# sile/libflate

Measured on AMD Instinct MI355X. Metric: gzip encode+decode throughput on 256 MiB synthetic text per GPU (uncompressed bytes through the round trip), higher is better.
Workload: dtype u8; 1 GPU; cfg2: gzip::Encoder (DefaultLz77Encoder, default options, mtime=0) + gzip::Decoder on TEXT(268435456 B) per GPU, write schedule S8K (8192-byte writes); bytes_per_gpu=268435456, schedule=S8K, compressed_bytes=129579521, parallelism=1 rank

## Files before the change

### libflate_amd/csrc/lfx_inflate_fast.hip

```cpp
#include <hip/hip_runtime.h>
#include <stdint.h>
#include <stdlib.h>

#include <type_traits>

#include "lfx_common.h"
#include "lfx_decode.h"

namespace lfx {

__constant__ uint16_t f_len_base[29] = {3,  4,  5,  6,  7,  8,  9,  10, 11,  13,  15,  17,  19,  23, 27,
                                        31, 35, 43, 51, 59, 67, 83, 99, 115, 131, 163, 195, 227, 258};
__constant__ uint8_t f_len_extra[29] = {0, 0, 0, 0, 0, 0, 0, 0, 1, 1, 1, 1, 2, 2, 2,
                                        2, 3, 3, 3, 3, 4, 4, 4, 4, 5, 5, 5, 5, 0};
__constant__ uint16_t f_dist_base[30] = {1,    2,    3,    4,    5,    7,    9,    13,    17,    25,
                                         33,   49,   65,   97,   129,  193,  257,  385,   513,   769,
                                         1025, 1537, 2049, 3073, 4097, 6145, 8193, 12289, 16385, 24577};
__constant__ uint8_t f_dist_extra[30] = {0, 0, 0, 0, 1, 1, 2, 2,  3,  3,  4,  4,  5,  5,  6,
                                         6, 7, 7, 8, 8, 9, 9, 10, 10, 11, 11, 12, 12, 13, 13};
__constant__ uint8_t f_clen_order[19] = {16, 17, 18, 0, 8, 7, 9, 6, 10, 5, 11, 4, 12, 3, 13, 2, 14, 1, 15};
constexpr uint32_t f_clen_order_c(uint32_t k) {
    constexpr uint8_t o[19] = {16, 17, 18, 0, 8, 7, 9, 6, 10, 5, 11, 4, 12, 3, 13, 2, 14, 1, 15};
    return o[k];
}
// ... 1057 lines not shown
                __syncthreads();
                uint32_t rounds = 0, no = 0, flag = 4;
                int32_t rr = INT32_MAX;
                uint64_t exitpos = ~0ull, decoded_from = ~0ull;
                for (;;) {
                    const uint64_t st = s_start[tid];
                    if (tid < nl && st != ~0ull) {
                        if (st != decoded_from) {
                            const int r = lane_count_reach(T, in, nb, st, tid + 1 == nl ? e : my_bound, no, rr, exitpos);
                            flag = r == 1 ? 1 : r == 2 ? 2 : 0;
                            decoded_from = st;
                        }
                    } else flag = 4;
                    s_flag[tid] = flag; s_exit[tid] = exitpos;
                    __syncthreads();
                    bool changed = false;
                    if (tid + 1 < nl && flag == 0 && s_start[tid + 1] != exitpos) { s_start[tid + 1] = exitpos; changed = true; }
                    rounds++;
                    const int any = __syncthreads_or(changed ? 1 : 0);
                    if (!any || rounds >= 64) break;
                }
                if (rounds >= 64) { fail = true; break; }
                if (tid < nl && s_flag[tid] != 0) atomicMin(&s_eob, tid);
                __syncthreads();
                uint32_t eobl = s_eob;
                if (eobl == 0xFFFFFFFFu) eobl = nl - 1;
                else if (s_flag[eobl] != 1) { fail = true; break; }
                else closed = true;
                const uint64_t myno = tid <= eobl ? no : 0;
                uint64_t y = myno;
                for (int o = 1; o < 64; o <<= 1) {
                    const uint64_t c = __shfl_up(y, o);
                    if ((int)lane >= o) y += c;
                }
                if (lane == 63) s_sum[wave] = y;
                __syncthreads();
                uint64_t py = 0, tot = 0;
                for (uint32_t w = 0; w < NT / 64; ++w) { const uint64_t s = s_sum[w]; py += w < wave ? s : 0; tot += s; }
                long long m = tid <= eobl && rr != INT32_MAX ? (long long)(produced + py + y - myno) + (long long)rr : INT64_MAX;
                for (int o = 32; o; o >>= 1) { const long long c = __shfl_xor(m, o); m = c < m ? c : m; }
                if (lane == 0) s_min[wave] = m;
                const uint64_t last_exit = s_exit[eobl];
                __syncthreads();
                for (uint32_t w = 0; w < NT / 64; ++w) { const long long c = s_min[w]; reach = c < reach ? c : reach; }
                produced += tot;
                if (closed) blk_end = last_exit;
                else if (last_exit <= w0 || last_exit >= end_bits) fail = true;
                else w0 = last_exit;
                __syncthreads();
            }
            if (fail) { produced = blk_out; break; }
        }
        if (blk_end <= cur || blk_end > end_bits) { produced = blk_out; break; }
        nblocks++;
        cur = blk_end;
        if (bfinal) { status = WALK_FINAL; break; }
        if (job.stop_bit && cur >= job.stop_bit) { status = WALK_STOP; break; }
        __syncthreads();
    }
    if (tid == 0) {
        WalkResult r;
        r.end_bit = cur; r.n_out = produced; r.stuck_bit = blk_bit; r.stuck_out = blk_out;
        r.reach = reach; r.status = status; r.nblocks = nblocks;
        results[blockIdx.x] = r;
    }
}

constexpr uint32_t MAX_UNITS = 8;

template <int NT = SCAN_THREADS>
__device__ __forceinline__ void blk_units_tail(const uint32_t tid, const BlkEmit &job, const BlkLanes *L, const int64_t reach,
                                               uint32_t cut_code, const uint64_t cut_pos, BlkUnits *U, const uint32_t unit_target,
                                               const uint32_t free_shift, const uint64_t t_begin, const uint64_t t_hdr) {
    const uint64_t t_dec = clock64();
    __shared__ int64_t s_wmin[NT / 64];
    const uint32_t lane = tid & 63, wave = tid >> 6;
    int64_t sfx = reach;
    for (int o = 1; o < 64; o <<= 1) {
        const int64_t y = __shfl_down(sfx, o);
        if (lane + o < 64 && y < sfx) sfx = y;
    }
    if (lane == 0) s_wmin[wave] = sfx;
    __syncthreads();
    int64_t later = __shfl_down(sfx, 1);
    if (lane == 63) later = INT64_MAX;
    for (uint32_t w = wave + 1; w < NT / 64; ++w) { const int64_t y = s_wmin[w]; if (y < later) later = y; }
    if (cut_code != 0xFFFFFFFFu && later < (int64_t)cut_pos) cut_code = 0xFFFFFFFFu;
    __shared__ uint32_t s_cut_code[NT];
    __shared__ uint64_t s_cut_pos[NT];
    s_cut_code[tid] = cut_code;
    s_cut_pos[tid] = cut_pos;
    __shared__ uint64_t s_legal[NT / 64];
    const uint64_t legal = __ballot(cut_code != 0xFFFFFFFFu);
    if (lane == 0) s_legal[wave] = legal;
    __syncthreads();
    const uint64_t t_cut = clock64();
    if (tid == 0) {
        uint32_t nu = 0, last = 0;
        uint32_t want_units = (job.n_codes + unit_target / 2) / unit_target;
        if (want_units < 1) want_units = 1;
        if (want_units > MAX_UNITS) want_units = MAX_UNITS;
        const uint32_t tol = job.n_codes / (2 * want_units);
        U->code0[0] = 0; U->out0[0] = 0;
        for (uint32_t b = 1; b < want_units; ++b) {
            const uint32_t ideal = (uint32_t)((uint64_t)job.n_codes * b / want_units);
            uint32_t l0 = (uint32_t)((uint64_t)job.nlanes * b / want_units);
            if (l0 >= NT) l0 = NT - 1;
            int up = -1, dn = -1;
            for (uint32_t w = l0 >> 6; w < NT / 64 && up < 0; ++w) {
                uint64_t m = s_legal[w];
                if (w == (l0 >> 6)) m &= ~0ull << (l0 & 63);
                if (m) up = (int)(w * 64 + (uint32_t)__builtin_ctzll(m));
            }
            for (int w = (int)(l0 >> 6); w >= 0 && dn < 0; --w) {
                uint64_t m = s_legal[w];
                if (w == (int)(l0 >> 6)) m &= (l0 & 63) ? ~0ull >> (64 - (l0 & 63)) : 0ull;
                if (m) dn = w * 64 + 63 - __builtin_clzll(m);
            }
            int pick = -1;
            uint32_t best = 0xFFFFFFFFu;
            if (up >= 0) { const uint32_t cc = s_cut_code[up]; const uint32_t d = cc > ideal ? cc - ideal : ideal - cc; if (d < best) { best = d; pick = up; } }
            if (dn >= 0) { const uint32_t cc = s_cut_code[dn]; const uint32_t d = cc > ideal ? cc - ideal : ideal - cc; if (d < best) { best = d; pick = dn; } }
            if (pick < 0 || best > tol) continue;
            const uint32_t cc = s_cut_code[pick];
            if (cc == 0 || cc <= last || cc >= job.n_codes) continue;
            nu++;
            U->code0[nu] = cc; U->out0[nu] = s_cut_pos[pick];
            last = cc;
        }
        nu++;
        U->code0[nu] = job.n_codes; U->out0[nu] = job.n_out;
        U->n = nu;
        uint32_t fn = 0;
        uint32_t fwant = (uint32_t)(job.n_out >> free_shift);
        fwant = fwant < 1 ? 1 : fwant > MAX_FREE_UNITS ? MAX_FREE_UNITS : fwant;
        U->fcode0[0] = 0; U->fout0[0] = 0;
        for (uint32_t b = 1; b < fwant; ++b) {
            const uint32_t l = (uint32_t)((uint64_t)job.nlanes * b / fwant);
            if (l == 0 || l >= job.nlanes) continue;
            const uint32_t cc = L->code_off[l];
            if (cc <= U->fcode0[fn] || cc >= job.n_codes) continue;
            fn++;
            U->fcode0[fn] = cc; U->fout0[fn] = L->out_off[l];
        }
        fn++;
        U->fcode0[fn] = job.n_codes; U->fout0[fn] = job.n_out;
        U->fn = fn;
        U->cyc[0] = (uint32_t)(t_hdr - t_begin); U->cyc[1] = (uint32_t)(t_dec - t_hdr);
        U->cyc[2] = (uint32_t)(t_cut - t_dec); U->cyc[3] = (uint32_t)(clock64() - t_cut);
    }
}

__device__ __forceinline__ void blk_flag_reach(uint32_t tid, int64_t reach, uint64_t hist, uint32_t *__restrict__ flags,
                                               uint32_t *__restrict__ job_flags) {
    __shared__ uint32_t s_fl;
    if (tid == 0) s_fl = 0;
    __syncthreads();
    if (reach < -(int64_t)hist) atomicOr(&s_fl, 1u);
    else if (reach < 0) atomicOr(&s_fl, 2u);
    __syncthreads();
    if (tid == 0 && s_fl) {
        const uint32_t f = s_fl;
        if ((f & 1u) && job_flags) job_flags[blockIdx.x] = 1u;
        if ((__atomic_load_n(&flags[0], __ATOMIC_RELAXED) & f) != f) atomicOr(&flags[0], f);
    }
}

template <bool RING, int NT = SCAN_THREADS>
__global__ __launch_bounds__(NT, RING ? 4 : 8) void blk_emit_kernel(const uint8_t *__restrict__ in, uint64_t nbytes,
                                                                const BlkEmit *__restrict__ jobs,
                                                                const BlkLanes *__restrict__ lanes,
                                                                uint32_t *__restrict__ codes,
                                                                uint32_t *__restrict__ flags,
                                                                BlkUnits *__restrict__ units, uint32_t unit_target, uint32_t free_shift,
                                                                uint32_t *__restrict__ job_flags,
                                                                const FastTabs *__restrict__ tabs) {
    __shared__ FastTabs T;
    __shared__ __attribute__((aligned(4))) uint8_t lens[640];
    __shared__ uint32_t hdr[8];
    __shared__ uint64_t hdr64[2];
    extern __shared__ uint32_t emit_stage[];
    __shared__ uint32_t s_ring[RING ? NT * RING_STRIDE : 1];
    const uint32_t tid = threadIdx.x;
    const BlkEmit job = jobs[blockIdx.x];
    BlkUnits *U = &units[blockIdx.x];
    if (job.placed) return;
    if (job.btype == 0) {
        if (tid == 0) {
            U->n = 1; U->code0[0] = 0; U->code0[1] = 0; U->out0[0] = 0; U->out0[1] = job.n_out;
            U->fn = 1; U->fcode0[0] = 0; U->fcode0[1] = 0; U->fout0[0] = 0; U->fout0[1] = job.n_out;
        }
        return;
    }
    const uint64_t t_begin = clock64();
    if (tabs) {
        const uint32_t *srcw = (const uint32_t *)&tabs[job.cand];
        uint32_t *dst = (uint32_t *)&T;
        constexpr uint32_t TW = sizeof(FastTabs) / 4, TPER = (TW + NT - 1) / NT;
        uint32_t tv[TPER];
#pragma unroll
        for (uint32_t k = 0; k < TPER; ++k) tv[k] = srcw[min(tid + k * NT, TW - 1)];
#pragma unroll
        for (uint32_t k = 0; k < TPER; ++k) if (tid + k * NT < TW) dst[tid + k * NT] = tv[k];
        __syncthreads();
    } else parse_header<NT>(in, nbytes, job.start_bit, T, lens, hdr, hdr64, tid);
    const uint64_t t_hdr = clock64();
    const BlkLanes *L = &lanes[job.cand];
    int64_t reach = INT64_MAX;
    uint32_t cut_code = 0xFFFFFFFFu;
    uint64_t cut_pos = 0;
    if (tid < job.nlanes) {
        const uint64_t st = L->start[tid];
        const uint64_t lim = tid + 1 < job.nlanes ? L->start[tid + 1] : (job.end_limit ? job.end_limit : ~0ull >> 1);
        uint32_t nc = 0, cc = 0, co = 0;
        const uint64_t out0 = L->out_off[tid];
        uint64_t no = out0, endpos;
        if (RING)
            lane_decode<true>(T, in, nbytes, st, lim, nc, no, codes + job.code_off + L->code_off[tid], reach, endpos, cc, co,
                              s_ring + tid * RING_STRIDE, emit_stage + tid * EMIT_STRIDE);
        else
            lane_decode_fifo<true>(T, in, nbytes, st, lim, nc, no, codes + job.code_off + L->code_off[tid], reach, endpos, cc, co,
                                   emit_stage + tid * EMIT_STRIDE);
        if (cc < nc) { cut_code = L->code_off[tid] + cc; cut_pos = out0 + co; }
    }
    blk_flag_reach(tid, reach, job.hist, flags, job_flags);
    blk_units_tail<NT>(tid, job, L, reach, cut_code, cut_pos, U, unit_target, free_shift, t_begin, t_hdr);
}



__global__ __launch_bounds__(SCAN_THREADS) void blk_place_kernel(const BlkEmit *__restrict__ jobs, const BlkLanes *__restrict__ lanes,
                                                                  const BlkLanesX *__restrict__ lanesx, const uint32_t *__restrict__ temp,
                                                                  uint32_t *__restrict__ codes, uint32_t *__restrict__ flags,
                                                                  BlkUnits *__restrict__ units, uint32_t unit_target, uint32_t free_shift,
                                                                  uint32_t *__restrict__ job_flags) {
    const uint32_t tid = threadIdx.x, lane = tid & 63;
    const BlkEmit job = jobs[blockIdx.x];
    if (!job.placed) return;
    const uint64_t t_begin = clock64();
    BlkUnits *U = &units[blockIdx.x];
    const BlkLanes *L = &lanes[job.cand];
    const BlkLanesX *X = &lanesx[job.cand];
    const bool live = tid < job.nlanes;
    const uint32_t my_head = live ? X->n_head[tid] : 0u, my_rest = live ? X->n_rest[tid] : 0u, my_at = X->rest_at[tid];
    const uint32_t my_off = L->code_off[tid];
    const uint32_t *src0 = temp + job.temp_off + (uint64_t)(tid & ~63u) * job.cap;
    uint32_t *dst0 = codes + job.code_off;
    constexpr uint32_t DEEP = 8;
    const uint32_t j0 = blockIdx.y * 32u;
    for (uint32_t j = j0; j < j0 + 32u; j += 2) {
        uint32_t nh[2], n[2], at[2];
        const uint32_t *src[2];
        uint32_t *dst[2];
#pragma unroll
        for (uint32_t q = 0; q < 2; ++q) {
            nh[q] = (uint32_t)__shfl((int)my_head, (int)(j + q));
            n[q] = nh[q] + (uint32_t)__shfl((int)my_rest, (int)(j + q));
            at[q] = (uint32_t)__shfl((int)my_at, (int)(j + q));
            src[q] = src0 + (uint64_t)(j + q) * job.cap;
            dst[q] = dst0 + (uint32_t)__shfl((int)my_off, (int)(j + q));
        }
        const uint32_t nmax = n[0] > n[1] ? n[0] : n[1];
        for (uint32_t base = 0; base < nmax; base += 64 * DEEP) {
            uint32_t v[2][DEEP];
#pragma unroll
            for (uint32_t q = 0; q < 2; ++q)
#pragma unroll
                for (uint32_t k = 0; k < DEEP; ++k) {
                    const uint32_t i = base + k * 64 + lane;
                    const uint32_t si = i < nh[q] ? i : at[q] + (i - nh[q]);
                    v[q][k] = i < n[q] ? src[q][si] : 0u;
                }
#pragma unroll
            for (uint32_t q = 0; q < 2; ++q)
#pragma unroll
                for (uint32_t k = 0; k < DEEP; ++k) {
                    const uint32_t i = base + k * 64 + lane;
                    if (i < n[q]) dst[q][i] = v[q][k];
                }
        }
    }
    if (blockIdx.y != 0) return;
    const uint64_t t_hdr = clock64();
    int64_t reach = INT64_MAX;
    uint32_t cut_code = 0xFFFFFFFFu;
    uint64_t cut_pos = 0;
    if (live) {
        const uint64_t out0 = L->out_off[tid];
        const int32_t rr = X->reach[tid];
        if (rr != INT32_MAX) reach = (int64_t)out0 + (int64_t)rr;
        const uint32_t cc = X->cut_code[tid];
        if (cc != 0xFFFFFFFFu) { cut_code = my_off + cc; cut_pos = out0 + X->cut_out[tid]; }
    }
    blk_flag_reach(tid, reach, job.hist, flags, job_flags);
    blk_units_tail(tid, job, L, reach, cut_code, cut_pos, U, unit_target, free_shift, t_begin, t_hdr);
}

template <uint32_t THREADS>
struct M2 {
    static constexpr uint32_t WAVES = THREADS / 64;
    static constexpr uint32_t NC = 2 * THREADS;
    static constexpr uint32_t TILE = 4 * THREADS;
    static constexpr uint32_t RING = 32768 + TILE;
    static constexpr uint32_t PASSES = (TILE + 4 * THREADS - 1) / (4 * THREADS);
    static_assert(RING % 4 == 0 && TILE >= 258 && TILE < 0xFFFFu && RING + 64 < 65536, "tile");
};
constexpr uint32_t M2_THREADS = 256;
constexpr uint32_t M2_WIDE_THREADS = 1024;
constexpr uint32_t M2_FEW_JOBS = 4;
constexpr uint32_t M2_SYM_THREADS = 256;
constexpr uint32_t M2_DONE = 0xFFFFu;
#ifndef LFX_M2_PRIO_TILES
#define LFX_M2_PRIO_TILES 8
#endif
constexpr uint32_t M2_PRIO_TILES = LFX_M2_PRIO_TILES;

template <uint32_t RING> __device__ __forceinline__ uint32_t m2_wrap(uint32_t x) { return min(x, x - RING); }
template <uint32_t RING> __device__ __forceinline__ uint32_t m2_back(uint32_t idx, uint32_t d) {
    const uint32_t a = idx - d;
    return min(a, a + RING);
}

template <bool SYM, uint32_t THREADS>
struct M2Lds {
    using elem_t = typename std::conditional<SYM, uint16_t, uint8_t>::type;
    using G = M2<THREADS>;
    static constexpr uint32_t RING_BYTES = ((G::RING + 64) * (uint32_t)sizeof(elem_t) + 15u) & ~15u;
    static constexpr uint32_t P_BYTES = G::PASSES * 4 * THREADS * 2;
    static constexpr uint32_t XC_BYTES = (G::NC + 4) * 8;
    static constexpr uint32_t SW_BYTES = 2 * G::WAVES * 4;
    static constexpr uint32_t BYTES = RING_BYTES + P_BYTES + XC_BYTES + SW_BYTES;
};
template <bool SYM, uint32_t THREADS, bool DYN = false, bool DICT = false>
__device__ __forceinline__ void materialize2_body(const uint8_t *__restrict__ in, const BlkEmit *__restrict__ jobs,
                                                  const BlkUnits *__restrict__ units,
                                                  const uint32_t *__restrict__ codes,
                                                  typename std::conditional<SYM, uint16_t, uint8_t>::type *__restrict__ out,
                                                  uint32_t njobs, uint64_t *__restrict__ dbg,
                                                  const uint8_t *__restrict__ dict_end = nullptr) {
    using elem_t = typename std::conditional<SYM, uint16_t, uint8_t>::type;
    using G = M2<THREADS>;
    using LD = M2Lds<SYM, THREADS>;
    constexpr uint32_t WAVES = G::WAVES, TILE = G::TILE, RING = G::RING, PASSES = G::PASSES, NC = G::NC;
    constexpr uint32_t EPD = 4 / sizeof(elem_t);
    elem_t *ring;
    uint16_t *P;
    uint2 *XC;
    uint32_t *s_w;
    if constexpr (DYN) {
        extern __shared__ __attribute__((aligned(16))) uint8_t m2_dyn[];
        ring = (elem_t *)m2_dyn;
        P = (uint16_t *)(m2_dyn + LD::RING_BYTES);
        XC = (uint2 *)(m2_dyn + LD::RING_BYTES + LD::P_BYTES);
        s_w = (uint32_t *)(m2_dyn + LD::RING_BYTES + LD::P_BYTES + LD::XC_BYTES);
    } else {
        __shared__ __attribute__((aligned(16))) elem_t ring_s[RING + 64];
        __shared__ __attribute__((aligned(8))) uint16_t P_s[PASSES * 4 * THREADS];
        __shared__ __attribute__((aligned(16))) uint2 XC_s[G::NC + 4];
        __shared__ uint32_t s_w_s[2 * WAVES];
        ring = ring_s; P = P_s; XC = XC_s; s_w = s_w_s;
    }
    const uint32_t bidx = blockIdx.x % njobs, u = blockIdx.x / njobs;
    const BlkEmit job = jobs[bidx];
    const uint32_t tid = threadIdx.x, lane = tid & 63, wave = tid >> 6;
    if (job.btype == 0) {
        if (u != 0) return;
        elem_t *o = out + job.out_off;
        const uint8_t *src = in + (job.data_bit >> 3);
        for (uint64_t k = tid; k < job.n_out; k += THREADS) o[k] = src[k];
        return;
    }
    const BlkUnits *U = &units[bidx];
    if (u >= (SYM ? U->fn : U->n)) return;
    const uint32_t c0 = SYM ? U->fcode0[u] : U->code0[u], c1 = SYM ? U->fcode0[u + 1] : U->code0[u + 1];
    const uint64_t ob = SYM ? U->fout0[u] : U->out0[u];
    const uint64_t gbase = job.out_off + ob;
    elem_t *o = out + gbase;
    const uint32_t *cp = codes + job.code_off + c0;
    const uint32_t n = c1 - c0;
    const uint32_t hist = SYM ? 32768u : (u == 0 && job.preload) ? (uint32_t)(job.hist < 32768 ? job.hist : 32768) : 0;
    const uint32_t shift = (uint32_t)((gbase - hist) & (EPD - 1)) + hist;
    if constexpr (DICT && !SYM) {
        const uint64_t own = job.hist - job.dict_len;
        for (uint32_t k = tid; k < hist; k += THREADS) {
            const uint32_t back = hist - k;
            ring[shift - hist + k] = back <= own ? o[-(int64_t)back] : dict_end[(int64_t)own - (int64_t)back];
        }
    } else
    for (uint32_t k = tid; k < hist; k += THREADS)
        ring[shift - hist + k] = SYM ? (elem_t)(256 + k) : (elem_t)o[(int64_t)k - (int64_t)hist];
    if (tid < 4) XC[NC + tid] = make_uint2(0xFFFFFFFFu, 0u);
    uint64_t produced = 0, flushed = 0;
    uint32_t tr = shift;
    uint32_t fr = shift;
    uint32_t base = 0, ntiles = 0, nrounds = 0;
    uint32_t cw0 = 2 * tid < n ? cp[2 * tid] : 0u, cw1 = 2 * tid + 1 < n ? cp[2 * tid + 1] : 0u;
    const uint64_t t0 = dbg ? clock64() : 0;
    while (base < n) {
        if ((ntiles & (M2_PRIO_TILES - 1)) == 0) {
            switch (((ntiles / M2_PRIO_TILES) + u) & 3u) {
            case 0: __builtin_amdgcn_s_setprio(0); break;
            case 1: __builtin_amdgcn_s_setprio(1); break;
            case 2: __builtin_amdgcn_s_setprio(2); break;
            default: __builtin_amdgcn_s_setprio(3); break;
            }
        }
        ntiles++;
        const uint32_t i = base + 2 * tid;
        const uint32_t len0 = i < n ? ((cw0 & 0xFFFFu) ? cw0 >> 16 : 1u) : 0u;
        const uint32_t len1 = i + 1 < n ? ((cw1 & 0xFFFFu) ? cw1 >> 16 : 1u) : 0u;
        uint32_t x = wave_inclusive_sum(len0 + len1);
        if (lane == 63) s_w[wave] = x;
        __syncthreads();
        uint32_t tot = 0, cum[WAVES];
#pragma unroll
        for (uint32_t j = 0; j < WAVES; ++j) {
            const uint32_t wj = s_w[j];
            x += j < wave ? wj : 0u;
            tot += wj;
            cum[j] = tot;
        }
        *(uint4 *)&XC[2 * tid] = make_uint4(x - len1, cw0, x, cw1);
        if (tot > TILE) {
            const uint32_t cnt = (uint32_t)__popcll(__ballot(x - len1 <= TILE)) + (uint32_t)__popcll(__ballot(x <= TILE));
            if (lane == 0) s_w[WAVES + wave] = cnt;
        }
        __syncthreads();
        uint32_t take = NC, total = tot;
        if (tot > TILE) {
            take = 0;
#pragma unroll
            for (uint32_t j = 0; j < WAVES; ++j) take += s_w[WAVES + j];
            total = XC[take - 1].x;
        }
        const uint32_t j0 = 2 * tid + take, j1 = j0 + 1;
        const uint32_t rf0 = (j0 >= NC && base + j0 < n) ? cp[base + j0] : 0u;
        const uint32_t rf1 = (j1 >= NC && base + j1 < n) ? cp[base + j1] : 0u;
        uint32_t pp[PASSES][4];
        bool pend = false;
        auto round0 = [&](auto periodic_tag) {
        constexpr bool PERIODIC = decltype(periodic_tag)::value;
#pragma unroll
        for (uint32_t ps = 0; ps < PASSES; ++ps) {
            const uint32_t b = ps * 4 * THREADS + 4 * tid;
#pragma unroll
            for (uint32_t q = 0; q < 4; ++q) pp[ps][q] = M2_DONE;
            if (ps == 0 || __ballot(b < total)) {
                uint32_t k = 0;
#pragma unroll
                for (uint32_t j = 0; j + 1 < WAVES; ++j) k += cum[j] <= b ? 128u : 0u;
#pragma unroll
                for (uint32_t step = 64; step; step >>= 1) k += XC[k + step - 1].x <= b ? step : 0u;
                uint32_t src[4], dst[4], cwq[4];
                bool lit[4], fin[4];
#pragma unroll
                for (uint32_t q = 0; q < 4; ++q) {
                    const uint32_t bi = b + q;
                    if (q) k += bi >= cwq[q - 1] ? 1u : 0u;
                    const uint2 xc = XC[k];
                    const uint32_t d = xc.y & 0xFFFFu;
                    const uint32_t t = m2_wrap<RING>(tr + bi);
                    const bool in = bi < total;
                    lit[q] = d == 0;
                    uint32_t tgt = bi, tt = t;
                    if constexpr (PERIODIC) {
                        const uint32_t s0 = xc.x - (xc.y >> 16);
                        const uint32_t off = bi - s0;
                        if (d != 0 && off >= d) {
                            uint32_t r = off - d * (uint32_t)((float)off * __builtin_amdgcn_rcpf((float)d));
                            r = r >= d ? r - d : r;
                            tgt = s0 + r;
                            tt = m2_wrap<RING>(tr + tgt);
                        }
                    }
                    fin[q] = lit[q] || d > tgt;
                    src[q] = (d > tgt && in) ? m2_back<RING>(tt, d) : t;
                    dst[q] = in ? t : RING + (tid & 63u);
                    pp[ps][q] = (fin[q] || !in) ? M2_DONE : tgt - d;
                    cwq[q] = xc.x;
                    src[q] |= xc.y & 0xFFFF0000u;
                }
                uint32_t hv[4];
#pragma unroll
                for (uint32_t q = 0; q < 4; ++q) hv[q] = ring[src[q] & 0xFFFFu];
#pragma unroll
                for (uint32_t q = 0; q < 4; ++q) ring[dst[q]] = (elem_t)(lit[q] ? src[q] >> 16 : hv[q]);
                pend |= (pp[ps][0] & pp[ps][1] & pp[ps][2] & pp[ps][3]) != M2_DONE;
            }
            *(uint64_t *)&P[b] = (uint64_t)pp[ps][0] | (uint64_t)pp[ps][1] << 16 | (uint64_t)pp[ps][2] << 32 | (uint64_t)pp[ps][3] << 48;
        }
        };
        if (take * 8 < total) round0(std::true_type{}); else round0(std::false_type{});
        __syncthreads();
        while (__ballot(pend)) {
            nrounds++;
            if (pend) {
#pragma unroll
                for (uint32_t ps = 0; ps < PASSES; ++ps) {
                    const uint32_t b = ps * 4 * THREADS + 4 * tid;
                    if (ps && (pp[ps][0] & pp[ps][1] & pp[ps][2] & pp[ps][3]) == M2_DONE) continue;
                    uint32_t nx[4], hv[4], jj[4];
#pragma unroll
                    for (uint32_t q = 0; q < 4; ++q) {
                        jj[q] = pp[ps][q] != M2_DONE ? pp[ps][q] : b + q;
                        nx[q] = P[jj[q]];
                    }
                    asm volatile("" ::: "memory");
#pragma unroll
                    for (uint32_t q = 0; q < 4; ++q) hv[q] = ring[m2_wrap<RING>(tr + jj[q])];
#pragma unroll
                    for (uint32_t q = 0; q < 4; ++q) {
                        ring[m2_wrap<RING>(tr + b + q)] = (elem_t)hv[q];
                        pp[ps][q] = nx[q];
                    }
                    asm volatile("" ::: "memory");
                    *(uint64_t *)&P[b] = (uint64_t)nx[0] | (uint64_t)nx[1] << 16 | (uint64_t)nx[2] << 32 | (uint64_t)nx[3] << 48;
                }
                pend = false;
#pragma unroll
                for (uint32_t ps = 0; ps < PASSES; ++ps) pend |= (pp[ps][0] & pp[ps][1] & pp[ps][2] & pp[ps][3]) != M2_DONE;
            }
        }
        __syncthreads();
        const uint64_t upto = produced + total;
        base += take;
        const bool last = base >= n;
        if ((gbase + flushed) & (EPD - 1)) {
            uint32_t hb = EPD - (uint32_t)((gbase + flushed) & (EPD - 1));
            if (hb > upto - flushed) hb = (uint32_t)(upto - flushed);
            if (tid < hb) o[flushed + tid] = ring[m2_wrap<RING>(fr + tid)];
            flushed += hb;
            fr = m2_wrap<RING>(fr + hb);
        }
        const uint32_t ndw = (uint32_t)((upto - flushed) / EPD);
        uint32_t *o32 = (uint32_t *)(o + flushed);
        for (uint32_t k = tid; k < ndw; k += THREADS) o32[k] = *(const uint32_t *)&ring[m2_wrap<RING>(fr + EPD * k)];
        flushed += (uint64_t)EPD * ndw;
        fr = m2_wrap<RING>(fr + EPD * ndw);
        if (last) {
            const uint32_t rest = (uint32_t)(upto - flushed);
            if (tid < rest) o[flushed + tid] = ring[m2_wrap<RING>(fr + tid)];
            flushed = upto;
        }
        produced = upto;
        tr = m2_wrap<RING>(tr + total);
        cw0 = j0 < NC ? XC[j0].y : rf0;
        cw1 = j1 < NC ? XC[j1].y : rf1;
    }
    if (!SYM && dbg && tid == 0) {
        uint64_t *d = dbg + ((uint64_t)bidx * MAX_UNITS + u) * 8;
        d[0] = clock64() - t0; d[1] = ntiles; d[2] = nrounds; d[3] = 0; d[4] = n; d[5] = produced; d[6] = wall_clock64();
    }
}


template <uint32_t THREADS>
__global__ __launch_bounds__(THREADS) void blk_materialize2_kernel(const uint8_t *__restrict__ in,
                                                                   const BlkEmit *__restrict__ jobs,
                                                                   const BlkUnits *__restrict__ units,
                                                                   const uint32_t *__restrict__ codes,
                                                                   uint8_t *__restrict__ out, uint32_t njobs,
                                                                   uint64_t *__restrict__ dbg) {
    materialize2_body<false, THREADS>(in, jobs, units, codes, out, njobs, dbg);
}
template <uint32_t THREADS>
__global__ __launch_bounds__(THREADS) void blk_materialize2_dict_kernel(const uint8_t *__restrict__ in,
                                                                        const BlkEmit *__restrict__ jobs,
                                                                        const BlkUnits *__restrict__ units,
                                                                        const uint32_t *__restrict__ codes,
                                                                        uint8_t *__restrict__ out, uint32_t njobs,
                                                                        const uint8_t *__restrict__ dict_end) {
    materialize2_body<false, THREADS, false, true>(in, jobs, units, codes, out, njobs, nullptr, dict_end);
}

__global__ __launch_bounds__(1024) void window_chain_kernel(const uint16_t *__restrict__ sym,
                                                            const SymUnit *__restrict__ units, uint32_t nunits,
                                                            uint8_t *__restrict__ windows, const uint8_t *__restrict__ init_win) {
    extern __shared__ uint8_t wbuf[];
    uint8_t *prev = wbuf, *cur = wbuf + 32768;
    for (uint32_t i = threadIdx.x; i < 32768; i += 1024) prev[i] = init_win ? init_win[i] : (uint8_t)0;
    uint32_t sn[16];
    auto fetch = [&](uint32_t u) {
        if (u >= nunits) return;
        const SymUnit su = units[u];
#pragma unroll
        for (uint32_t k = 0; k < 8; ++k) {
            const uint32_t i = 4 * (threadIdx.x + 1024 * k);
            const uint64_t at = su.start + su.len - 32768 + i;
            const uint32_t s0 = sym[su.len + i >= 32768 ? at : 0];
            const uint32_t s1 = sym[su.len + i + 1 >= 32768 ? at + 1 : 0];
            const uint32_t s2 = sym[su.len + i + 2 >= 32768 ? at + 2 : 0];
            const uint32_t s3 = sym[su.len + i + 3 >= 32768 ? at + 3 : 0];
            sn[2 * k] = s0 | s1 << 16;
            sn[2 * k + 1] = s2 | s3 << 16;
        }
    };
    fetch(0);
    __syncthreads();
    for (uint32_t u = 0; u < nunits; ++u) {
        const uint64_t len = units[u].len;
        uint32_t sc[16];
#pragma unroll
        for (uint32_t k = 0; k < 16; ++k) sc[k] = sn[k];
        fetch(u + 1);
        uint32_t *wout = (uint32_t *)(windows + (uint64_t)u * 32768);
#pragma unroll
        for (uint32_t k = 0; k < 8; ++k) {
            const uint32_t i = 4 * (threadIdx.x + 1024 * k);
            uint32_t lb[4], sv[4];
            bool own[4];
#pragma unroll
            for (uint32_t q = 0; q < 4; ++q) {
                sv[q] = (sc[2 * k + (q >> 1)] >> (16 * (q & 1))) & 0xFFFFu;
                own[q] = len + i + q >= 32768;
                const uint32_t at = own[q] ? (sv[q] >= 256 ? sv[q] - 256 : 0u) : i + q + (uint32_t)len;
                lb[q] = prev[at];
            }
            uint32_t packed = 0;
#pragma unroll
            for (uint32_t q = 0; q < 4; ++q) packed |= ((own[q] && sv[q] < 256) ? sv[q] : lb[q]) << (8 * q);
            ((uint32_t *)cur)[i >> 2] = packed;
            wout[i >> 2] = packed;
        }
        __syncthreads();
        uint8_t *t = prev; prev = cur; cur = t;
    }
}

__host__ __device__ inline uint32_t wc_group(uint32_t nunits) {
    uint32_t g = 4;
    while (g * g < nunits && g < 64) ++g;
    return g;
}
__device__ __forceinline__ uint32_t unit_map_load(const uint16_t *__restrict__ sym, const SymUnit &su, uint32_t i) {
    return sym[su.len + i >= 32768 ? su.start + su.len - 32768 + i : 0];
}
__device__ __forceinline__ uint32_t unit_map_value(uint32_t loaded, const SymUnit &su, uint32_t i) {
    return su.len + i >= 32768 ? loaded : 256u + i + (uint32_t)su.len;
}
__global__ __launch_bounds__(1024) void window_compose_kernel(const uint16_t *__restrict__ sym,
                                                              const SymUnit *__restrict__ units, uint32_t nunits,
                                                              uint16_t *__restrict__ maps, uint32_t WC_GROUP) {
    extern __shared__ uint16_t mbuf[];
    uint16_t *prev = mbuf, *cur = mbuf + 32768;
    const uint32_t u0 = blockIdx.x * WC_GROUP, u1 = u0 + WC_GROUP < nunits ? u0 + WC_GROUP : nunits;
    if (u0 >= u1) return;
    uint32_t nx[16];
    auto load_unit = [&](const SymUnit &su) {
        if (su.len >= 32768) {
            const uint16_t *p = sym + (su.start + su.len - 32768) + threadIdx.x;
#pragma unroll
            for (uint32_t k = 0; k < 16; ++k) nx[k] = (uint32_t)p[1024 * (2 * k)] | (uint32_t)p[1024 * (2 * k + 1)] << 16;
        } else {
#pragma unroll
            for (uint32_t k = 0; k < 16; ++k)
                nx[k] = unit_map_load(sym, su, threadIdx.x + 1024 * (2 * k)) | unit_map_load(sym, su, threadIdx.x + 1024 * (2 * k + 1)) << 16;
        }
    };
    SymUnit sun = units[u0];
    load_unit(sun);
    for (uint32_t u = u0; u < u1; ++u) {
        const SymUnit su = sun;
        uint32_t sc[16];
#pragma unroll
        for (uint32_t k = 0; k < 16; ++k) sc[k] = nx[k];
        if (u + 1 < u1) {
            sun = units[u + 1];
            load_unit(sun);
        }
        uint16_t *mout = maps + (uint64_t)u * 32768;
        const bool first = u == u0;
#pragma unroll
        for (uint32_t h = 0; h < 4; ++h) {
            uint32_t sv[8], g[8];
#pragma unroll
            for (uint32_t j = 0; j < 8; ++j) {
                const uint32_t k = 8 * h + j;
                sv[j] = unit_map_value((sc[k >> 1] >> (16 * (k & 1))) & 0xFFFFu, su, threadIdx.x + 1024 * k);
                g[j] = prev[sv[j] >= 256 ? sv[j] - 256 : 0u];
            }
#pragma unroll
            for (uint32_t j = 0; j < 8; ++j) {
                const uint32_t k = 8 * h + j;
                const uint32_t v = (!first && sv[j] >= 256) ? g[j] : sv[j];
                cur[threadIdx.x + 1024 * k] = (uint16_t)v;
                mout[threadIdx.x + 1024 * k] = (uint16_t)v;
            }
        }
        __syncthreads();
        uint16_t *t = prev; prev = cur; cur = t;
    }
}
__device__ __forceinline__ void map_octet(const uint4 &q, uint32_t (&s8)[8]) {
    s8[0] = q.x & 0xFFFFu; s8[1] = q.x >> 16; s8[2] = q.y & 0xFFFFu; s8[3] = q.y >> 16;
    s8[4] = q.z & 0xFFFFu; s8[5] = q.z >> 16; s8[6] = q.w & 0xFFFFu; s8[7] = q.w >> 16;
}
__device__ __forceinline__ void window_step_bytes(const uint4 (&mq)[4], const uint8_t *prev, uint8_t *cur, uint8_t *gout) {
#pragma unroll
    for (uint32_t k = 0; k < 4; ++k) {
        const uint32_t o = threadIdx.x + 1024 * k;
        uint32_t s8[8], b8[8];
        map_octet(mq[k], s8);
#pragma unroll
        for (uint32_t j = 0; j < 8; ++j) b8[j] = prev[s8[j] >= 256 ? s8[j] - 256 : 0u];
        uint32_t lo = 0, hi = 0;
#pragma unroll
        for (uint32_t j = 0; j < 4; ++j) {
            lo |= ((s8[j] < 256 ? s8[j] : b8[j]) & 0xFFu) << (8 * j);
            hi |= ((s8[j + 4] < 256 ? s8[j + 4] : b8[j + 4]) & 0xFFu) << (8 * j);
        }
        *(uint2 *)(cur + 8 * o) = make_uint2(lo, hi);
        if (gout) *(uint2 *)(gout + 8 * o) = make_uint2(lo, hi);
    }
}
__global__ __launch_bounds__(1024) void window_groups_kernel(const uint16_t *__restrict__ maps, uint32_t nunits,
                                                             uint8_t *__restrict__ gwin, const uint8_t *__restrict__ init_win,
                                                             uint32_t WC_GROUP) {
    extern __shared__ __attribute__((aligned(16))) uint8_t wbuf[];
    uint8_t *prev = wbuf, *cur = wbuf + 32768;
    for (uint32_t i = threadIdx.x; i < 32768; i += 1024) prev[i] = init_win ? init_win[i] : (uint8_t)0;
    const uint32_t ngroups = (nunits + WC_GROUP - 1) / WC_GROUP;
    auto last_of = [&](uint32_t g) { return (g + 1) * WC_GROUP < nunits ? (g + 1) * WC_GROUP - 1 : nunits - 1; };
    uint4 nx[4];
    if (ngroups) {
        const uint4 *m = (const uint4 *)(maps + (uint64_t)last_of(0) * 32768);
#pragma unroll
        for (uint32_t k = 0; k < 4; ++k) nx[k] = m[threadIdx.x + 1024 * k];
    }
    __syncthreads();
    for (uint32_t g = 0; g < ngroups; ++g) {
        uint4 mq[4];
#pragma unroll
        for (uint32_t k = 0; k < 4; ++k) mq[k] = nx[k];
        if (g + 1 < ngroups) {
            const uint4 *m = (const uint4 *)(maps + (uint64_t)last_of(g + 1) * 32768);
#pragma unroll
            for (uint32_t k = 0; k < 4; ++k) nx[k] = m[threadIdx.x + 1024 * k];
        }
        window_step_bytes(mq, prev, cur, gwin + (uint64_t)g * 32768);
        __syncthreads();
        uint8_t *t = prev; prev = cur; cur = t;
    }
}
__global__ __launch_bounds__(1024) void window_apply_kernel(const uint16_t *__restrict__ maps, const uint8_t *__restrict__ gwin,
                                                            uint8_t *__restrict__ windows, const uint8_t *__restrict__ init_win,
                                                            uint32_t WC_GROUP) {
    __shared__ __attribute__((aligned(16))) uint8_t wl[32768];
    const uint32_t u = blockIdx.x, g = u / WC_GROUP;
    const uint8_t *w = g ? gwin + (uint64_t)(g - 1) * 32768 : init_win;
    const uint4 *m = (const uint4 *)(maps + (uint64_t)u * 32768);
    uint4 mq[4];
#pragma unroll
    for (uint32_t k = 0; k < 4; ++k) mq[k] = m[threadIdx.x + 1024 * k];
    {
        const uint4 z = make_uint4(0, 0, 0, 0);
        const uint4 *w16 = (const uint4 *)w;
        if (w && ((uint64_t)w & 15) == 0) {
            ((uint4 *)wl)[threadIdx.x] = w16[threadIdx.x];
            ((uint4 *)wl)[threadIdx.x + 1024] = w16[threadIdx.x + 1024];
        } else if (w) {
            for (uint32_t i = threadIdx.x; i < 32768; i += 1024) wl[i] = w[i];
        } else {
            ((uint4 *)wl)[threadIdx.x] = z;
            ((uint4 *)wl)[threadIdx.x + 1024] = z;
        }
    }
    __syncthreads();
    uint8_t *wout = windows + (uint64_t)u * 32768;
#pragma unroll
    for (uint32_t k = 0; k < 4; ++k) {
        const uint32_t o = threadIdx.x + 1024 * k;
        uint32_t s8[8], b8[8];
        map_octet(mq[k], s8);
#pragma unroll
        for (uint32_t j = 0; j < 8; ++j) b8[j] = wl[s8[j] >= 256 ? s8[j] - 256 : 0u];
        uint32_t lo = 0, hi = 0;
#pragma unroll
        for (uint32_t j = 0; j < 4; ++j) {
            lo |= ((s8[j] < 256 ? s8[j] : b8[j]) & 0xFFu) << (8 * j);
            hi |= ((s8[j + 4] < 256 ? s8[j + 4] : b8[j + 4]) & 0xFFu) << (8 * j);
        }
        *(uint2 *)(wout + 8 * o) = make_uint2(lo, hi);
    }
}

__global__ __launch_bounds__(1024) void window_rank_map_kernel(const uint16_t *__restrict__ maps, uint32_t nunits,
                                                               uint16_t *__restrict__ out_map, uint32_t WC_GROUP) {
    extern __shared__ __attribute__((aligned(16))) uint16_t mbuf2[];
    uint16_t *prev = mbuf2, *cur = mbuf2 + 32768;
    for (uint32_t i = threadIdx.x; i < 32768; i += 1024) prev[i] = (uint16_t)(256u + i);
    const uint32_t ngroups = (nunits + WC_GROUP - 1) / WC_GROUP;
    auto last_of = [&](uint32_t g) { return (g + 1) * WC_GROUP < nunits ? (g + 1) * WC_GROUP - 1 : nunits - 1; };
    uint4 nx[4];
    if (ngroups) {
        const uint4 *m = (const uint4 *)(maps + (uint64_t)last_of(0) * 32768);
#pragma unroll
        for (uint32_t k = 0; k < 4; ++k) nx[k] = m[threadIdx.x + 1024 * k];
    }
    __syncthreads();
    for (uint32_t g = 0; g < ngroups; ++g) {
        uint4 mq[4];
#pragma unroll
        for (uint32_t k = 0; k < 4; ++k) mq[k] = nx[k];
        if (g + 1 < ngroups) {
            const uint4 *m = (const uint4 *)(maps + (uint64_t)last_of(g + 1) * 32768);
#pragma unroll
            for (uint32_t k = 0; k < 4; ++k) nx[k] = m[threadIdx.x + 1024 * k];
        }
#pragma unroll
        for (uint32_t k = 0; k < 4; ++k) {
            const uint32_t o = threadIdx.x + 1024 * k;
            uint32_t s8[8], g8[8];
            map_octet(mq[k], s8);
#pragma unroll
            for (uint32_t j = 0; j < 8; ++j) g8[j] = prev[s8[j] >= 256 ? s8[j] - 256 : 0u];
#pragma unroll
            for (uint32_t j = 0; j < 8; ++j) s8[j] = s8[j] < 256 ? s8[j] : g8[j];
            *(uint4 *)(cur + 8 * o) = make_uint4(s8[0] | s8[1] << 16, s8[2] | s8[3] << 16, s8[4] | s8[5] << 16, s8[6] | s8[7] << 16);
        }
        __syncthreads();
        uint16_t *t = prev; prev = cur; cur = t;
    }
    for (uint32_t i = threadIdx.x; i < 32768; i += 1024) out_map[i] = prev[i];
}
__global__ __launch_bounds__(256) void bytes_to_map_kernel(const uint8_t *__restrict__ out, uint64_t len, uint16_t *__restrict__ map) {
    const uint32_t i = blockIdx.x * 256 + threadIdx.x;
    if (i >= 32768) return;
    map[i] = len + i >= 32768 ? (uint16_t)out[len + i - 32768] : (uint16_t)(256u + i + (uint32_t)len);
}
__global__ __launch_bounds__(1024) void window_ranks_kernel(const uint16_t *__restrict__ maps, uint32_t nranks, uint8_t *__restrict__ win) {
    extern __shared__ __attribute__((aligned(16))) uint8_t wbuf3[];
    uint8_t *prev = wbuf3, *cur = wbuf3 + 32768;
    for (uint32_t i = threadIdx.x; i < 32768; i += 1024) prev[i] = 0;
    uint4 nx[4];
    if (nranks) {
#pragma unroll
        for (uint32_t k = 0; k < 4; ++k) nx[k] = ((const uint4 *)maps)[threadIdx.x + 1024 * k];
    }
    __syncthreads();
    for (uint32_t r = 0; r < nranks; ++r) {
        uint4 mq[4];
#pragma unroll
        for (uint32_t k = 0; k < 4; ++k) mq[k] = nx[k];
        if (r + 1 < nranks) {
            const uint4 *m = (const uint4 *)(maps + (uint64_t)(r + 1) * 32768);
#pragma unroll
            for (uint32_t k = 0; k < 4; ++k) nx[k] = m[threadIdx.x + 1024 * k];
// ... 528 lines not shown
```

Before: 60.74 GB/s.

## Align materialize tiles to 4-element groups and flush output directly from registers

Each tile now starts at a 4-aligned ring position, so each thread owns one aligned group of 4 output elements. It writes that group to the ring as one packed store and stores the same register value straight to global output. This removes the separate flush loop that re-read the ring after a barrier, removes one __syncthreads per tile, drops the multi-pass P array and the ring's 64-element scratch pad, and shrinks usable tile capacity by the alignment offset. The risk is subtle correctness at unaligned edges: partial groups go through byte-wise fallback stores and now rely on the next tile rewriting overlapping elements, while the sentinel changes to 0x7FFFFFFF and comparisons become signed.

```diff
diff --git a/libflate_amd/csrc/lfx_inflate_fast.hip b/libflate_amd/csrc/lfx_inflate_fast.hip
--- a/libflate_amd/csrc/lfx_inflate_fast.hip
+++ b/libflate_amd/csrc/lfx_inflate_fast.hip
@@ -1383,8 +1383,7 @@
     static constexpr uint32_t NC = 2 * THREADS;
     static constexpr uint32_t TILE = 4 * THREADS;
     static constexpr uint32_t RING = 32768 + TILE;
-    static constexpr uint32_t PASSES = (TILE + 4 * THREADS - 1) / (4 * THREADS);
-    static_assert(RING % 4 == 0 && TILE >= 258 && TILE < 0xFFFFu && RING + 64 < 65536, "tile");
+    static_assert(RING % 4 == 0 && TILE - 3 >= 258 && TILE < 0xFFFFu && RING < 65536, "tile");
 };
 constexpr uint32_t M2_THREADS = 256;
 constexpr uint32_t M2_WIDE_THREADS = 1024;
@@ -1406,8 +1405,8 @@
 struct M2Lds {
     using elem_t = typename std::conditional<SYM, uint16_t, uint8_t>::type;
     using G = M2<THREADS>;
-    static constexpr uint32_t RING_BYTES = ((G::RING + 64) * (uint32_t)sizeof(elem_t) + 15u) & ~15u;
-    static constexpr uint32_t P_BYTES = G::PASSES * 4 * THREADS * 2;
+    static constexpr uint32_t RING_BYTES = (G::RING * (uint32_t)sizeof(elem_t) + 15u) & ~15u;
+    static constexpr uint32_t P_BYTES = 4 * THREADS * 2;
     static constexpr uint32_t XC_BYTES = (G::NC + 4) * 8;
     static constexpr uint32_t SW_BYTES = 2 * G::WAVES * 4;
     static constexpr uint32_t BYTES = RING_BYTES + P_BYTES + XC_BYTES + SW_BYTES;
@@ -1422,8 +1421,16 @@
     using elem_t = typename std::conditional<SYM, uint16_t, uint8_t>::type;
     using G = M2<THREADS>;
     using LD = M2Lds<SYM, THREADS>;
-    constexpr uint32_t WAVES = G::WAVES, TILE = G::TILE, RING = G::RING, PASSES = G::PASSES, NC = G::NC;
-    constexpr uint32_t EPD = 4 / sizeof(elem_t);
+    constexpr uint32_t WAVES = G::WAVES, TILE = G::TILE, RING = G::RING, NC = G::NC;
+    using group_t = typename std::conditional<SYM, uint2, uint32_t>::type;
+    auto pack = [](const uint32_t (&v)[4]) -> group_t {
+        if constexpr (SYM) return make_uint2(v[0] | v[1] << 16, v[2] | v[3] << 16);
+        else return v[0] | v[1] << 8 | v[2] << 16 | v[3] << 24;
+    };
+    auto unpack = [](const group_t &g, uint32_t q) -> elem_t {
+        if constexpr (SYM) return (elem_t)((q < 2 ? g.x : g.y) >> (16 * (q & 1)));
+        else return (elem_t)(g >> (8 * q));
+    };
     elem_t *ring;
     uint16_t *P;
     uint2 *XC;
@@ -1435,8 +1442,8 @@
         XC = (uint2 *)(m2_dyn + LD::RING_BYTES + LD::P_BYTES);
         s_w = (uint32_t *)(m2_dyn + LD::RING_BYTES + LD::P_BYTES + LD::XC_BYTES);
     } else {
-        __shared__ __attribute__((aligned(16))) elem_t ring_s[RING + 64];
-        __shared__ __attribute__((aligned(8))) uint16_t P_s[PASSES * 4 * THREADS];
+        __shared__ __attribute__((aligned(16))) elem_t ring_s[RING];
+        __shared__ __attribute__((aligned(8))) uint16_t P_s[4 * THREADS];
         __shared__ __attribute__((aligned(16))) uint2 XC_s[G::NC + 4];
         __shared__ uint32_t s_w_s[2 * WAVES];
         ring = ring_s; P = P_s; XC = XC_s; s_w = s_w_s;
@@ -1460,7 +1467,7 @@
     const uint32_t *cp = codes + job.code_off + c0;
     const uint32_t n = c1 - c0;
     const uint32_t hist = SYM ? 32768u : (u == 0 && job.preload) ? (uint32_t)(job.hist < 32768 ? job.hist : 32768) : 0;
-    const uint32_t shift = (uint32_t)((gbase - hist) & (EPD - 1)) + hist;
+    const uint32_t shift = (uint32_t)((gbase - hist) & 3u) + hist;
     if constexpr (DICT && !SYM) {
         const uint64_t own = job.hist - job.dict_len;
         for (uint32_t k = tid; k < hist; k += THREADS) {
@@ -1470,10 +1477,9 @@
     } else
     for (uint32_t k = tid; k < hist; k += THREADS)
         ring[shift - hist + k] = SYM ? (elem_t)(256 + k) : (elem_t)o[(int64_t)k - (int64_t)hist];
-    if (tid < 4) XC[NC + tid] = make_uint2(0xFFFFFFFFu, 0u);
-    uint64_t produced = 0, flushed = 0;
+    if (tid < 4) XC[NC + tid] = make_uint2(0x7FFFFFFFu, 0u);
+    uint64_t produced = 0;
     uint32_t tr = shift;
-    uint32_t fr = shift;
     uint32_t base = 0, ntiles = 0, nrounds = 0;
     uint32_t cw0 = 2 * tid < n ? cp[2 * tid] : 0u, cw1 = 2 * tid + 1 < n ? cp[2 * tid + 1] : 0u;
     const uint64_t t0 = dbg ? clock64() : 0;
@@ -1487,6 +1493,7 @@
             }
         }
         ntiles++;
+        const uint32_t a = tr & 3u, tra = tr - a, cap = TILE - a;
         const uint32_t i = base + 2 * tid;
         const uint32_t len0 = i < n ? ((cw0 & 0xFFFFu) ? cw0 >> 16 : 1u) : 0u;
         const uint32_t len1 = i + 1 < n ? ((cw1 & 0xFFFFu) ? cw1 >> 16 : 1u) : 0u;
@@ -1502,13 +1509,13 @@
             cum[j] = tot;
         }
         *(uint4 *)&XC[2 * tid] = make_uint4(x - len1, cw0, x, cw1);
-        if (tot > TILE) {
-            const uint32_t cnt = (uint32_t)__popcll(__ballot(x - len1 <= TILE)) + (uint32_t)__popcll(__ballot(x <= TILE));
+        if (tot > cap) {
+            const uint32_t cnt = (uint32_t)__popcll(__ballot(x - len1 <= cap)) + (uint32_t)__popcll(__ballot(x <= cap));
             if (lane == 0) s_w[WAVES + wave] = cnt;
         }
         __syncthreads();
         uint32_t take = NC, total = tot;
-        if (tot > TILE) {
+        if (tot > cap) {
             take = 0;
 #pragma unroll
             for (uint32_t j = 0; j < WAVES; ++j) take += s_w[WAVES + j];
@@ -1517,32 +1524,30 @@
         const uint32_t j0 = 2 * tid + take, j1 = j0 + 1;
         const uint32_t rf0 = (j0 >= NC && base + j0 < n) ? cp[base + j0] : 0u;
         const uint32_t rf1 = (j1 >= NC && base + j1 < n) ? cp[base + j1] : 0u;
-        uint32_t pp[PASSES][4];
+        const uint32_t g = m2_wrap<RING>(tra + 4 * tid);
+        uint32_t pp[4];
+        group_t gv;
         bool pend = false;
         auto round0 = [&](auto periodic_tag) {
         constexpr bool PERIODIC = decltype(periodic_tag)::value;
-#pragma unroll
-        for (uint32_t ps = 0; ps < PASSES; ++ps) {
-            const uint32_t b = ps * 4 * THREADS + 4 * tid;
-#pragma unroll
-            for (uint32_t q = 0; q < 4; ++q) pp[ps][q] = M2_DONE;
-            if (ps == 0 || __ballot(b < total)) {
+            {
+                const uint32_t b = (uint32_t)max((int32_t)(4 * tid) - (int32_t)a, 0);
                 uint32_t k = 0;
 #pragma unroll
                 for (uint32_t j = 0; j + 1 < WAVES; ++j) k += cum[j] <= b ? 128u : 0u;
 #pragma unroll
                 for (uint32_t step = 64; step; step >>= 1) k += XC[k + step - 1].x <= b ? step : 0u;
-                uint32_t src[4], dst[4], cwq[4];
+                uint32_t src[4], cwq[4];
                 bool lit[4], fin[4];
 #pragma unroll
                 for (uint32_t q = 0; q < 4; ++q) {
-                    const uint32_t bi = b + q;
-                    if (q) k += bi >= cwq[q - 1] ? 1u : 0u;
+                    const uint32_t bi = 4 * tid + q - a;
+                    if (q) k += (int32_t)bi >= (int32_t)cwq[q - 1] ? 1u : 0u;
                     const uint2 xc = XC[k];
                     const uint32_t d = xc.y & 0xFFFFu;
-                    const uint32_t t = m2_wrap<RING>(tr + bi);
+                    const uint32_t t = g + q;
                     const bool in = bi < total;
-                    lit[q] = d == 0;
+                    lit[q] = d == 0 && in;
                     uint32_t tgt = bi, tt = t;
                     if constexpr (PERIODIC) {
                         const uint32_t s0 = xc.x - (xc.y >> 16);
@@ -1556,8 +1561,7 @@
                     }
                     fin[q] = lit[q] || d > tgt;
                     src[q] = (d > tgt && in) ? m2_back<RING>(tt, d) : t;
-                    dst[q] = in ? t : RING + (tid & 63u);
-                    pp[ps][q] = (fin[q] || !in) ? M2_DONE : tgt - d;
+                    pp[q] = (fin[q] || !in) ? M2_DONE : tgt - d + a;
                     cwq[q] = xc.x;
                     src[q] |= xc.y & 0xFFFF0000u;
                 }
@@ -1565,65 +1569,48 @@
 #pragma unroll
                 for (uint32_t q = 0; q < 4; ++q) hv[q] = ring[src[q] & 0xFFFFu];
 #pragma unroll
-                for (uint32_t q = 0; q < 4; ++q) ring[dst[q]] = (elem_t)(lit[q] ? src[q] >> 16 : hv[q]);
-                pend |= (pp[ps][0] & pp[ps][1] & pp[ps][2] & pp[ps][3]) != M2_DONE;
+                for (uint32_t q = 0; q < 4; ++q) hv[q] = lit[q] ? src[q] >> 16 : hv[q];
+                gv = pack(hv);
+                *(group_t *)&ring[g] = gv;
+                pend = (pp[0] & pp[1] & pp[2] & pp[3]) != M2_DONE;
             }
-            *(uint64_t *)&P[b] = (uint64_t)pp[ps][0] | (uint64_t)pp[ps][1] << 16 | (uint64_t)pp[ps][2] << 32 | (uint64_t)pp[ps][3] << 48;
-        }
+            *(uint64_t *)&P[4 * tid] = (uint64_t)pp[0] | (uint64_t)pp[1] << 16 | (uint64_t)pp[2] << 32 | (uint64_t)pp[3] << 48;
         };
         if (take * 8 < total) round0(std::true_type{}); else round0(std::false_type{});
         __syncthreads();
         while (__ballot(pend)) {
             nrounds++;
             if (pend) {
-#pragma unroll
-                for (uint32_t ps = 0; ps < PASSES; ++ps) {
-                    const uint32_t b = ps * 4 * THREADS + 4 * tid;
-                    if (ps && (pp[ps][0] & pp[ps][1] & pp[ps][2] & pp[ps][3]) == M2_DONE) continue;
-                    uint32_t nx[4], hv[4], jj[4];
-#pragma unroll
-                    for (uint32_t q = 0; q < 4; ++q) {
-                        jj[q] = pp[ps][q] != M2_DONE ? pp[ps][q] : b + q;
-                        nx[q] = P[jj[q]];
-                    }
-                    asm volatile("" ::: "memory");
-#pragma unroll
-                    for (uint32_t q = 0; q < 4; ++q) hv[q] = ring[m2_wrap<RING>(tr + jj[q])];
-#pragma unroll
-                    for (uint32_t q = 0; q < 4; ++q) {
-                        ring[m2_wrap<RING>(tr + b + q)] = (elem_t)hv[q];
-                        pp[ps][q] = nx[q];
-                    }
-                    asm volatile("" ::: "memory");
-                    *(uint64_t *)&P[b] = (uint64_t)nx[0] | (uint64_t)nx[1] << 16 | (uint64_t)nx[2] << 32 | (uint64_t)nx[3] << 48;
+                uint32_t nx[4], hv[4], jj[4];
+#pragma unroll
+                for (uint32_t q = 0; q < 4; ++q) {
+                    jj[q] = pp[q] != M2_DONE ? pp[q] : 4 * tid + q;
+                    nx[q] = P[jj[q]];
                 }
-                pend = false;
-#pragma unroll
-                for (uint32_t ps = 0; ps < PASSES; ++ps) pend |= (pp[ps][0] & pp[ps][1] & pp[ps][2] & pp[ps][3]) != M2_DONE;
+                asm volatile("" ::: "memory");
+#pragma unroll
+                for (uint32_t q = 0; q < 4; ++q) hv[q] = ring[m2_wrap<RING>(tra + jj[q])];
+                gv = pack(hv);
+                *(group_t *)&ring[g] = gv;
+#pragma unroll
+                for (uint32_t q = 0; q < 4; ++q) pp[q] = nx[q];
+                asm volatile("" ::: "memory");
+                *(uint64_t *)&P[4 * tid] = (uint64_t)nx[0] | (uint64_t)nx[1] << 16 | (uint64_t)nx[2] << 32 | (uint64_t)nx[3] << 48;
+                pend = (pp[0] & pp[1] & pp[2] & pp[3]) != M2_DONE;
             }
         }
-        __syncthreads();
-        const uint64_t upto = produced + total;
         base += take;
         const bool last = base >= n;
-        if ((gbase + flushed) & (EPD - 1)) {
-            uint32_t hb = EPD - (uint32_t)((gbase + flushed) & (EPD - 1));
-            if (hb > upto - flushed) hb = (uint32_t)(upto - flushed);
-            if (tid < hb) o[flushed + tid] = ring[m2_wrap<RING>(fr + tid)];
-            flushed += hb;
-            fr = m2_wrap<RING>(fr + hb);
-        }
-        const uint32_t ndw = (uint32_t)((upto - flushed) / EPD);
-        uint32_t *o32 = (uint32_t *)(o + flushed);
-        for (uint32_t k = tid; k < ndw; k += THREADS) o32[k] = *(const uint32_t *)&ring[m2_wrap<RING>(fr + EPD * k)];
-        flushed += (uint64_t)EPD * ndw;
-        fr = m2_wrap<RING>(fr + EPD * ndw);
-        if (last) {
-            const uint32_t rest = (uint32_t)(upto - flushed);
-            if (tid < rest) o[flushed + tid] = ring[m2_wrap<RING>(fr + tid)];
-            flushed = upto;
-        }
-        produced = upto;
+        const uint32_t lo = a > produced ? a - (uint32_t)produced : 0u, hi = a + total;
+        const uint32_t gb = 4 * tid;
+        elem_t *og = o + ((int64_t)produced - (int64_t)a + (int64_t)gb);
+        if (gb >= lo && gb + 4 <= hi) *(group_t *)og = gv;
+        else if (gb < hi && (gb < lo || last)) {
+#pragma unroll
+            for (uint32_t q = 0; q < 4; ++q)
+                if (gb + q >= lo && gb + q < hi) og[q] = unpack(gv, q);
+        }
+        produced += total;
         tr = m2_wrap<RING>(tr + total);
         cw0 = j0 < NC ? XC[j0].y : rf0;
         cw1 = j1 < NC ? XC[j1].y : rf1;
```

Result: no change. 61.28 GB/s, median of 6 (+0.9%).
